# jasonleebrown/machisplin

Hardware: AMD Instinct MI355X
Metric: grid Mcells/s (ensemble+TPS predict) + TPS-solve GFLOP/s (higher is better)
Workload: dtype f64; 1 GPU; cfg3: 5000 stations, 3 covariates, 10000x10000 grid, 6-model ensemble + TPS residual correction; stations=5000, covariates=3 x float32 planes resident in HBM, rf_trees=500, tps_mode=global (one fit on all stations, GCV lambda, V73:748-753), parallelism=rowband1 + bcast(coef) + 1 all-gather

## Files before the change

include/machisplin_hip.h:

```cpp
#ifndef MACHISPLIN_HIP_H
#define MACHISPLIN_HIP_H

#include <stdint.h>

#if defined(__GNUC__)
#define MHS_API __attribute__((visibility("default")))
#else
#define MHS_API
#endif

#ifdef __cplusplus
extern "C" {
#endif

enum {
    MHS_OK = 0,
    MHS_ERR_INVALID = 1,
    MHS_ERR_HIP = 2,
    MHS_ERR_NODEVICE = 3,
    MHS_ERR_NUMERIC = 4,
    MHS_ERR_ALLOC = 5
};

enum { MHS_F64 = 0, MHS_F32 = 1, MHS_I16 = 2 };
// ... 88 lines not shown
MHS_API int mhs_nnet_fit_many(int count, const double *const *X, const double *const *y, const int64_t *n, int p, int size,
                              double *const *wts, int maxit, double abstol, double reltol, double *value, int *counts,
                              int *fail);
MHS_API int mhs_nnet_load(const double *wts, int p, int size, double y_scale, double y_shift,
                          mhs_model **out);
MHS_API int mhs_earth_load(const double *coef, const int32_t *dirs, const double *cuts, int nterms,
                           int p, mhs_model **out);
MHS_API int mhs_svr_load(const double *alpha, const double *sv, int64_t nsv, int p, double b,
                         double sigma, const double *x_center, const double *x_scale,
                         double y_center, double y_scale, mhs_model **out);
MHS_API int mhs_gbm_load(double init_f, int64_t n_trees, const int64_t *tree_offsets,
                         const int32_t *split_var, const double *split_val, const int32_t *left,
                         const int32_t *right, const int32_t *missing, int p, mhs_model **out);
MHS_API int mhs_gbm_grow_many(int count, const double *const *X, const double *const *y, const int64_t *n, int p,
                              const int32_t *const *bags, const int64_t *bag_size, int n_new, int interaction_depth,
                              int n_minobsinnode, double shrinkage, int first_call, double *const *F, double *init_f,
                              int64_t *const *tree_offsets, int32_t *const *split_var, double *const *split_val,
                              int32_t *const *left, int32_t *const *right, int32_t *const *missing);
MHS_API int mhs_gbm_grow_many_reduction(int count, const double *const *X, const double *const *y, const int64_t *n, int p,
                                        const int32_t *const *bags, const int64_t *bag_size, int n_new, int interaction_depth,
                                        int n_minobsinnode, double shrinkage, int first_call, double *const *F, double *init_f,
                                        int64_t *const *tree_offsets, int32_t *const *split_var, double *const *split_val,
                                        int32_t *const *left, int32_t *const *right, int32_t *const *missing,
                                        double *const *error_reduction);
MHS_API int mhs_rf_load(int64_t n_trees, const int64_t *tree_offsets, const int32_t *left,
                        const int32_t *right, const int32_t *status, const int32_t *best_var,
                        const double *split, const double *node_pred, int p, mhs_model **out);
MHS_API int mhs_rf_fit_many(int count, const double *const *X, const double *const *y, const int64_t *n, int p,
                            int n_trees, int mtry, int nodesize, const int32_t *const *inbag,
                            const uint64_t *const *seeds, mhs_model **models_out, double *const *oob_pred,
                            int32_t *const *oob_count, double *const *inc_node_purity);
MHS_API int mhs_rf_get(const mhs_model *m, int64_t *n_nodes, int32_t *left, int32_t *right, int32_t *status,
                       int32_t *best_var, double *split, double *node_pred, int64_t *tree_offsets);
MHS_API int mhs_rf_importance_many(int count, const mhs_model *const *models, const double *const *X,
                                   const double *const *y, const int64_t *n, int p, const int32_t *const *inbag,
                                   const uint64_t *const *perm_seeds, int n_perm, double *const *inc_mse,
                                   double *const *inc_mse_sd, double *const *tree_delta);
#define MHS_EARTH_MAX_NK 65
#define MHS_EARTH_STOP_CONSTANT 1
#define MHS_EARTH_STOP_NK 2
#define MHS_EARTH_STOP_NONE 3
#define MHS_EARTH_STOP_THRESH 4
#define MHS_EARTH_STOP_RSQ 5
#define MHS_EARTH_STOP_GRSQ 6
MHS_API int mhs_earth_fit_many(int count, const double *const *X, const double *const *y, const int64_t *n, int p,
                               int nk , double thresh, double penalty, int minspan, int endspan,
                               mhs_model **models_out);
MHS_API int mhs_earth_get(const mhs_model *m, int *n_selected, int *n_forward, int *stop_reason, double *coef,
                          int32_t *dirs, double *cuts, int32_t *forward_dirs, double *forward_cuts, double *forward_rss,
                          int32_t *selected, double *rss_per_subset, double *gcv_per_subset, int32_t *prune_terms,
                          double *stats);
MHS_API int mhs_model_free(mhs_model *m);

typedef struct mhs_stack {
    const void *data;
    int32_t n_layers;
    int32_t dtype;
    int64_t plane_stride;
    int64_t ld;
    double nodata;
} mhs_stack;

MHS_API int mhs_predict_dev(const mhs_model *m, const mhs_grid *g, const mhs_stack *covars,
                            int64_t r0, int64_t r1, int64_t c0, int64_t c1, double weight,
                            int accumulate, double *out_dev, int64_t ld, void *stream);
MHS_API int mhs_members_predict_dev(const mhs_model *const *models, const double *weights, int n_models,
// ... 226 lines not shown
```

machisplin_amd/_lib.py:

```python
from __future__ import annotations

import atexit
import ctypes as C
import os
import threading

_HERE = os.path.dirname(os.path.abspath(__file__))
LIB_PATH = os.path.join(_HERE, "libmachisplin_hip.so")

OK, ERR_INVALID, ERR_HIP, ERR_NODEVICE, ERR_NUMERIC, ERR_ALLOC = range(6)
F64, F32, I16 = 0, 1, 2
GCV_FIELDS, GCV_CONVERGED = 0, 1


class MhsError(RuntimeError):
    def __init__(self, code: int, msg: str):
        super().__init__(f"[mhs status {code}] {msg}")
        self.code = code


class Grid(C.Structure):
    _fields_ = [("xmin", C.c_double), ("ymax", C.c_double), ("xres", C.c_double),
                ("yres", C.c_double), ("nrow", C.c_int64), ("ncol", C.c_int64)]

# ... 85 lines not shown
    "mhs_tps_predict_points": (C.c_int, [_vp, _vp, _i64, _vp]),
    "mhs_tps_sigma2": (C.c_int, [_vp, _dp]),
    "mhs_tps_se_max_n": (C.c_int, [_i64, C.POINTER(_i64)]),
    "mhs_tps_se_build_mode": (C.c_int, [C.c_int]),
    "mhs_tps_se_info": (C.c_int, [_vp, C.POINTER(C.c_int), C.POINTER(C.c_double), C.POINTER(_i64)]),
    "mhs_tps_predict_se_points": (C.c_int, [_vp, _vp, _i64, C.c_double, _vp]),
    "mhs_tps_predict_se_grid": (C.c_int, [_vp, C.POINTER(Grid), _i64, _i64, _i64, _i64, C.c_double, _vp]),
    "mhs_tps_predict_se_grid_dev": (C.c_int, [_vp, C.POINTER(Grid), _i64, _i64, _i64, _i64, C.c_double, _vp, _i64, _vp]),
    "mhs_tps_eval_mode": (C.c_int, [C.c_int]),
    "mhs_tps_eval_plan": (C.c_int, [_vp, C.POINTER(C.c_int), C.POINTER(C.c_int), C.POINTER(_i64), C.POINTER(_i64)]),
    "mhs_lm_load": (C.c_int, [_vp, C.c_int, C.POINTER(_vp)]),
    "mhs_lm_fit": (C.c_int, [_vp, _vp, _i64, C.c_int, _vp]),
    "mhs_svr_fit": (C.c_int, [_vp, _vp, _i64, C.c_int, C.c_double, C.c_double, C.c_double, C.c_double, _i64, _vp, _vp, _vp, _vp,
                              _vp, _vp, _vp]),
    "mhs_nnet_fit": (C.c_int, [_vp, _vp, _i64, C.c_int, C.c_int, _vp, C.c_int, C.c_double, C.c_double, _vp, _vp, _vp]),
    "mhs_svr_fit_many": (C.c_int, [C.c_int, _vp, _vp, _vp, C.c_int, _vp, C.c_double, C.c_double, C.c_double, _i64, _i64, _vp, _vp, _vp,
                                   _vp, _vp, _vp, _vp, _vp]),
    "mhs_nnet_fit_many": (C.c_int, [C.c_int, _vp, _vp, _vp, C.c_int, C.c_int, _vp, C.c_int, C.c_double, C.c_double, _vp, _vp, _vp]),
    "mhs_nnet_load": (C.c_int, [_vp, C.c_int, C.c_int, C.c_double, C.c_double, C.POINTER(_vp)]),
    "mhs_earth_load": (C.c_int, [_vp, _vp, _vp, C.c_int, C.c_int, C.POINTER(_vp)]),
    "mhs_earth_fit_many": (C.c_int, [C.c_int, _vp, _vp, _vp, C.c_int, C.c_int, C.c_double, C.c_double, C.c_int, C.c_int, _vp]),
    "mhs_earth_get": (C.c_int, [_vp, _vp, _vp, _vp, _vp, _vp, _vp, _vp, _vp, _vp, _vp, _vp, _vp, _vp, _vp]),
    "mhs_svr_load": (C.c_int, [_vp, _vp, _i64, C.c_int, C.c_double, C.c_double, _vp, _vp, C.c_double,
                               C.c_double, C.POINTER(_vp)]),
    "mhs_gbm_load": (C.c_int, [C.c_double, _i64, _vp, _vp, _vp, _vp, _vp, _vp, C.c_int, C.POINTER(_vp)]),
    "mhs_gbm_grow_many": (C.c_int, [C.c_int, _vp, _vp, _vp, C.c_int, _vp, _vp, C.c_int, C.c_int, C.c_int, C.c_double, C.c_int, _vp, _vp,
                                    _vp, _vp, _vp, _vp, _vp, _vp]),
    "mhs_gbm_grow_many_reduction": (C.c_int, [C.c_int, _vp, _vp, _vp, C.c_int, _vp, _vp, C.c_int, C.c_int, C.c_int, C.c_double, C.c_int, _vp,
                                              _vp, _vp, _vp, _vp, _vp, _vp, _vp, _vp]),
    "mhs_rf_load": (C.c_int, [_i64, _vp, _vp, _vp, _vp, _vp, _vp, _vp, C.c_int, C.POINTER(_vp)]),
    "mhs_rf_fit_many": (C.c_int, [C.c_int, _vp, _vp, _vp, C.c_int, C.c_int, C.c_int, C.c_int, _vp, _vp, _vp, _vp, _vp, _vp]),
    "mhs_rf_get": (C.c_int, [_vp, _vp, _vp, _vp, _vp, _vp, _vp, _vp, _vp]),
    "mhs_rf_importance_many": (C.c_int, [C.c_int, _vp, _vp, _vp, _vp, C.c_int, _vp, _vp, C.c_int, _vp, _vp, _vp]),
    "mhs_model_free": (C.c_int, [_vp]),
    "mhs_predict_dev": (C.c_int, [_vp, C.POINTER(Grid), C.POINTER(Stack), _i64, _i64, _i64, _i64,
                                  C.c_double, C.c_int, _vp, _i64, _vp]),
    "mhs_members_predict_dev": (C.c_int, [C.POINTER(_vp), _dp, C.c_int, C.POINTER(Grid), C.POINTER(Stack), C.c_int64, C.c_int64,
                                          C.c_int64, C.c_int64, C.c_int, C.c_void_p, C.c_int64, C.c_void_p]),
    "mhs_ensemble_predict_dev": (C.c_int, [C.POINTER(_vp), _dp, C.c_int, C.c_double, C.POINTER(Grid),
                                           C.POINTER(Stack), _i64, _i64, _i64, _i64, _vp, _i64, _vp]),
    "mhs_ensemble_predict": (C.c_int, [C.POINTER(_vp), _dp, C.c_int, C.c_double, C.POINTER(Grid),
                                       C.POINTER(Stack), _i64, _i64, _i64, _i64, _vp]),
    "mhs_predict_points": (C.c_int, [_vp, _vp, _i64, _vp]),
    "mhs_gbm_staged_points": (C.c_int, [_vp, _vp, _i64, C.c_int, _vp]),
    "mhs_model_info": (C.c_int, [_vp, _vp, _vp, _vp]),
    "mhs_gbm_probe_last": (C.c_int, [_vp, _vp, _vp]),
    "mhs_residual_points": (C.c_int, [_vp, _vp, C.c_int, C.c_double, _vp, _vp, _i64, _vp]),
    "mhs_scale_add_dev": (C.c_int, [_vp, C.c_double, _vp, _vp, _i64, _vp]),
    "mhs_mess_create": (C.c_int, [_vp, _i64, C.c_int, C.POINTER(_vp)]),
    "mhs_mess_free": (C.c_int, [_vp]),
    "mhs_mess_grid_dev": (C.c_int, [_vp, C.POINTER(Grid), C.POINTER(Stack), _i64, _i64, _i64, _i64, _vp, _i64, _vp, _i64, _vp]),
    "mhs_mess_grid": (C.c_int, [_vp, C.POINTER(Grid), C.POINTER(Stack), _i64, _i64, _i64, _i64, _vp, _vp]),
    "mhs_mess_points": (C.c_int, [_vp, _vp, _i64, _vp, _vp]),
    "mhs_terrain_max_radius": (C.c_int, []),
    "mhs_terrain_dev": (C.c_int, [C.POINTER(Grid), C.POINTER(Stack), C.c_int, C.POINTER(TerrainUnits), _i64, _i64, _i64, _i64, C.c_uint,
                                  _vp, C.c_int, _i64, _i64, _vp]),
    "mhs_relief_dev": (C.c_int, [C.POINTER(Grid), C.POINTER(Stack), C.c_int, C.POINTER(TerrainUnits), C.c_int, _i64, _i64, _i64, _i64,
                                 C.c_uint, _vp, C.c_int, _i64, _i64, _vp]),
    "mhs_geomorphon_dev": (C.c_int, [C.POINTER(Grid), C.POINTER(Stack), C.c_int, C.POINTER(TerrainUnits), C.c_int, C.c_double, _i64, _i64,
                                     _i64, _i64, _vp, _i64, _vp]),
    "mhs_terrain": (C.c_int, [C.POINTER(Grid), C.POINTER(Stack), C.c_int, C.POINTER(TerrainUnits), _i64, _i64, _i64, _i64, C.c_uint, _vp,
                              C.c_int]),
    "mhs_relief": (C.c_int, [C.POINTER(Grid), C.POINTER(Stack), C.c_int, C.POINTER(TerrainUnits), C.c_int, _i64, _i64, _i64, _i64, C.c_uint,
                             _vp, C.c_int]),
    "mhs_geomorphon": (C.c_int, [C.POINTER(Grid), C.POINTER(Stack), C.c_int, C.POINTER(TerrainUnits), C.c_int, C.c_double, _i64, _i64, _i64,
                                 _i64, _vp]),
# ... 132 lines not shown
```

machisplin_amd/csrc/forest.hip:

```cpp
#include <type_traits>
#include <algorithm>
#include <cmath>
#include <cstdio>
#include <cstdlib>
#include <cstring>
#include <vector>
#include "ensemble_int.h"
#include "devmath.h"

namespace mhs {

constexpr int RF_COARSE_BYTES = LUT_COARSE * (int)sizeof(float);
constexpr unsigned RF_LEAF_WORD = 0xffffff00u;
typedef unsigned uint2v __attribute__((ext_vector_type(2)));
typedef unsigned uint4v __attribute__((ext_vector_type(4)));
__device__ __forceinline__ uint2v lds_u2(unsigned a) { return *(__attribute__((address_space(3))) const uint2v *)(uintptr_t)a; }
__device__ __forceinline__ unsigned lds_u32(unsigned a) { return *(__attribute__((address_space(3))) const unsigned *)(uintptr_t)a; }
__device__ __forceinline__ double lds_f64(unsigned a) { return *(__attribute__((address_space(3))) const double *)(uintptr_t)a; }

__host__ __device__ constexpr int rf_walks(int code) { return code >= 3 ? code + 2 : (1 << code); }


template <int R>
__device__ __forceinline__ void rf_lane_cells(const PredGeom &g, int64_t i0, int strips, int (&row)[R], int (&col)[R], bool (&live)[R]) {
    const int64_t total = (int64_t)g.nr * g.nc;
    const int64_t part = (total + R - 1) / R;
#pragma unroll
    for (int c = 0; c < R; ++c) {
        if (strips) {
            const int64_t sr = i0 / g.nc;
            col[c] = (int)(i0 - sr * g.nc);
            const int64_t r = sr * R + c;
            live[c] = r < g.nr;
            row[c] = (int)(live[c] ? r : g.nr - 1);
        } else {
            int64_t i = i0 + c * part;
            live[c] = i0 < part && i < total;
            if (i >= total) i = total - 1;
            row[c] = (int)(i / g.nc); col[c] = (int)(i - (int64_t)row[c] * g.nc);
        }
    }
}
static int64_t rf_lane_count(const PredGeom &g, int R, int strips) {
    const int64_t total = (int64_t)g.nr * g.nc;
    return strips ? (((int64_t)g.nr + R - 1) / R) * g.nc : (total + R - 1) / R;
}
static int rf_strips(const PredGeom &g, int R) { return g.nr >= 4 * R; }

constexpr int RF_ENTRY_BATCHES = 16;
constexpr int RF_PREFIX_MAX_P = 12;
template <int R>
__device__ __forceinline__ void rf_prefix_entries(unsigned (&entry)[RF_ENTRY_BATCHES], const uint2 *__restrict__ gnodes,
                                                  const int *__restrict__ tree_off, int n_trees, int p, const char *smem,
                                                  unsigned lane_base, const bool (&na)[R]) {
    const int lane = threadIdx.x & 63;
    int mn[RF_PREFIX_MAX_P], mx[RF_PREFIX_MAX_P];
#pragma unroll
    for (int v = 0; v < 12; ++v) {
        mn[v] = 0x7fffffff; mx[v] = -1;
        if (v < p) {
            int a = 0x7fffffff, b = -1;
#pragma unroll
            for (int c = 0; c < R; ++c)
                if (!na[c]) {
                    const int rk = (int)(*(const unsigned *)(smem + lane_base + (unsigned)(v * R + c) * 4u) >> 8);
                    a = min(a, rk); b = max(b, rk);
                }
#pragma unroll
            for (int q = 32; q > 0; q >>= 1) { a = min(a, __shfl_xor(a, q)); b = max(b, __shfl_xor(b, q)); }
            mn[v] = __builtin_amdgcn_readfirstlane(a); mx[v] = __builtin_amdgcn_readfirstlane(b);
        }
    }
#pragma unroll
    for (int b = 0; b < RF_ENTRY_BATCHES; ++b) {
        if (b * 64 < n_trees) {
            const int t = b * 64 + lane;
            bool walking = t < n_trees;
            const int o = tree_off[min(t, n_trees - 1)];
            unsigned nd = 0u, plen = 0u, term = 0u;
            while (__builtin_amdgcn_ballot_w64(walking)) {
                if (walking) {
                    const uint2 rec = gnodes[o + (int)nd];
                    if (rec.x == RF_LEAF_WORD) { term = 1u; walking = false; }
// ... 132 lines not shown
        for (int c = 0; c < R; ++c) {
            acc[c] = acc[c] + pending[c];
            pending[c] = glval[o + (int)((node[c] - boff) >> 3)];
        }
        __syncthreads();
        o = o1; o1 = o2; o2 = o3; o3 = o4;
        levels = levels1; levels1 = levels2;
        shallow = shallow1; shallow1 = shallow2;
    }
#pragma unroll
    for (int c = 0; c < R; ++c) {
        acc[c] = acc[c] + pending[c];
        if (live[c])
            emit(out, (int64_t)row[c] * g.ld_out + col[c], na[c] ? NAN : acc[c] / (double)n_trees, weight, accumulate);
    }
}

__device__ __forceinline__ void lds_wait_ge(unsigned addr, unsigned target) {
    for (;;) {
        unsigned v;
        asm volatile("ds_read_b32 %0, %1\n\ts_waitcnt lgkmcnt(0)" : "=v"(v) : "v"(addr) : "memory");
        if ((unsigned)__builtin_amdgcn_readfirstlane((int)v) >= target) break;
        __builtin_amdgcn_s_sleep(2);
    }
}
__device__ __forceinline__ void lds_signal(unsigned addr) {
    if ((threadIdx.x & 63) == 0) asm volatile("ds_add_u32 %0, %1" :: "v"(addr), "v"(1u) : "memory");
    else asm volatile("" ::: "memory");
}

__device__ __forceinline__ void glds16(const void *gsrc, unsigned lds_dst) {
    asm volatile("s_mov_b32 m0, %1\n\ts_nop 0\n\tglobal_load_lds_dwordx4 %0, off" :: "v"(gsrc), "s"(lds_dst) : "memory");
}
enum { RF_LD_PREFIX = 1 };

template <int LOG2R, bool K64, int STRIDE>
__global__ __launch_bounds__(1024) void rf_walk_ld_kernel(const uint2 *__restrict__ gnodes,
                                                          const double *__restrict__ glval,
                                                          const int *__restrict__ tree_off,
                                                          const int *__restrict__ depth,
                                                          const void *__restrict__ sorted,
                                                          const int *__restrict__ sorted_off, int n_trees,
                                                          int p, StackDev s, PredGeom g,
                                                          double weight, int accumulate,
                                                          double *__restrict__ out, const int *__restrict__ dmin, int strips, int flags,
                                                          const int *__restrict__ axis_rank, int axis_ncol) {
    constexpr int R = rf_walks(LOG2R), NL = 1, WALKERS = 16 - NL;
    constexpr unsigned TREE_BYTES = 3u * STRIDE;
    static_assert(TREE_BYTES >= (unsigned)RF_COARSE_BYTES && 2 * STRIDE <= 65535, "buffer bases inside the 16-bit immediate offsets");
    constexpr unsigned CNT = TREE_BYTES;
    extern __shared__ __attribute__((aligned(16))) char smem[];
    float *coarse = (float *)smem;
    const unsigned stride = (unsigned)(p * R) | 1u;
    const unsigned lane_base = TREE_BYTES + 32u + threadIdx.x * stride * 4u;
    if ((unsigned)(uintptr_t)(__attribute__((address_space(3))) char *)smem != 0u) __builtin_trap();
    const bool loader = threadIdx.x >= 64 * WALKERS;
    const int64_t i0 = (int64_t)blockIdx.x * (64 * WALKERS) + (loader ? threadIdx.x - 64 * WALKERS : threadIdx.x);
    int row[R], col[R];
    bool na[R], live[R];
    if (strips == 2) {
        const int wave = (int)(threadIdx.x >> 6), lane_ = (int)(threadIdx.x & 63u);
        const int64_t tile = (int64_t)blockIdx.x * WALKERS + (loader ? wave - WALKERS : wave);
        const int tiles_x = (g.nc + 15) / 16;
        const int64_t ty = tile / tiles_x;
        const int tx = (int)(tile - ty * tiles_x);
#pragma unroll
        for (int c = 0; c < R; ++c) {
            const int64_t r = ty * (4 * R) + (lane_ >> 4) * R + c;
            const int cc = tx * 16 + (lane_ & 15);
            live[c] = r < g.nr && cc < g.nc;
            row[c] = (int)min(r, (int64_t)g.nr - 1); col[c] = min(cc, g.nc - 1);
        }
    } else
    rf_lane_cells<R>(g, i0, strips, row, col, live);
#pragma unroll
    for (int c = 0; c < R; ++c) na[c] = false;
    for (int j = 0; j < p; ++j) {
        float r[R];
        if (axis_rank && j >= s.C && !s.all_from_planes) {
#pragma unroll
            for (int c = 0; c < R; ++c)
                r[c] = (float)(j == s.C ? axis_rank[g.c0 + col[c]] : axis_rank[(int64_t)axis_ncol + g.r0 + row[c]]);
        } else if constexpr (K64) lut_ranks_t<R, 1024, double>(j, (const double *)sorted, sorted_off, (double *)coarse, s, g, row, col, na, r);
        else lut_ranks_t<R, 1024, float>(j, (const float *)sorted, sorted_off, coarse, s, g, row, col, na, r);
#pragma unroll
        for (int c = 0; c < R; ++c) *(unsigned *)(smem + lane_base + (unsigned)(j * R + c) * 4u) = (unsigned)r[c] << 8;
    }
    unsigned entry[RF_ENTRY_BATCHES];
#pragma unroll
    for (int b = 0; b < RF_ENTRY_BATCHES; ++b) entry[b] = 0u;
    if (!loader && (flags & RF_LD_PREFIX) && p <= RF_PREFIX_MAX_P && n_trees <= 64 * RF_ENTRY_BATCHES)
        rf_prefix_entries<R>(entry, gnodes, tree_off, n_trees, p, smem, lane_base, na);
    __syncthreads();
    if (threadIdx.x < 8) *(unsigned *)(smem + CNT + threadIdx.x * 4u) = 0u;
    __syncthreads();
    if (loader) {
        constexpr int PF = (STRIDE + 1023) / 1024;
        static_assert(PF <= 25, "one named register quad per piece below");
        const unsigned lane16 = (threadIdx.x & 63u) * 16u;
        uint4 r0, r1, r2, r3, r4, r5, r6, r7, r8, r9, r10, r11, r12, r13, r14, r15, r16, r17, r18, r19, r20, r21, r22, r23, r24;
        const char *src = nullptr;
#define MHS_RF_ALL(F) F(0) F(1) F(2) F(3) F(4) F(5) F(6) F(7) F(8) F(9) F(10) F(11) F(12) F(13) F(14) F(15) F(16) F(17) F(18) F(19) F(20) \
                      F(21) F(22) F(23) F(24)
#define MHS_RF_LOAD(Q) if constexpr (Q < PF) r##Q = *(const uint4 *)(src + (size_t)Q * 1024u);
#define MHS_RF_STORE(Q) if constexpr (Q < PF) *(uint4 *)(smem + slot * (unsigned)STRIDE + (unsigned)Q * 1024u + lane16) = r##Q;
#define MHS_RF_REQUEST(U) { \
            src = (const char *)(gnodes + tree_off[(U)]) + lane16; \
            MHS_RF_ALL(MHS_RF_LOAD) }
        {
            MHS_RF_REQUEST(0)
            for (int u = 0; u < n_trees; u += 2) {
                unsigned slot = (unsigned)u % 3u;
                if (u >= 3) lds_wait_ge(CNT + 16u + 4u * slot, (unsigned)WALKERS * (unsigned)(u / 3));
                MHS_RF_ALL(MHS_RF_STORE)
                lds_signal(CNT + 4u * slot);
                if (u + 2 < n_trees) MHS_RF_REQUEST(u + 2)
                if (u + 1 < n_trees) {
                    slot = (unsigned)(u + 1) % 3u;
                    if (u + 1 >= 3) lds_wait_ge(CNT + 16u + 4u * slot, (unsigned)WALKERS * (unsigned)((u + 1) / 3));
                    {
                        const char *dsrc = (const char *)(gnodes + tree_off[u + 1]) + lane16;
#pragma unroll
                        for (int q = 0; q < PF; ++q)
                            glds16(dsrc + (size_t)q * 1024u, (unsigned)__builtin_amdgcn_readfirstlane((int)(slot * (unsigned)STRIDE + (unsigned)q * 1024u)));
                        asm volatile("s_waitcnt vmcnt(0)" ::: "memory");
                    }
                    lds_signal(CNT + 4u * slot);
                }
            }
            return;
        }
#undef MHS_RF_REQUEST
#undef MHS_RF_STORE
#undef MHS_RF_LOAD
#undef MHS_RF_ALL
        return;
    }
    constexpr int PD = 6;
    double acc[R], pend[PD][R];
#pragma unroll
    for (int c = 0; c < R; ++c) {
        acc[c] = 0.0;
#pragma unroll
        for (int k = 0; k < PD; ++k) pend[k][c] = 0.0;
    }
    unsigned staged[3] = {0u, 0u, 0u};
    int ocur = 0;
    unsigned wcur = 0u;
    double tpcur = 0.0;
    const int lane = threadIdx.x & 63;
    auto step = [&](auto slot_tag, auto pidx_tag, const int t, const unsigned k3) {
        constexpr int SLOT = decltype(slot_tag)::value, PIDX = decltype(pidx_tag)::value;
        if ((t & 63) == 0) {
            unsigned ecur = 0u;
#pragma unroll
            for (int b = 0; b < RF_ENTRY_BATCHES; ++b) if ((t >> 6) == b) ecur = entry[b];
            const int tl = min(t + lane, n_trees - 1);
            ocur = tree_off[tl];
            const int dcur = depth[tl], mcur = dmin ? dmin[tl] : dcur;
            const int plen = (int)((ecur >> 16) & 0x7FFFu);
            const int levels = (ecur >> 31) ? 0 : dcur - plen, shallow = max(mcur - plen, 0);
            const int c0 = min(shallow, levels - 1), cnt = levels - 1 - c0;
            wcur = ((ecur & 0xFFFFu) << 3) | (levels > 0 ? ((unsigned)c0 << 19) | ((unsigned)cnt << 25) | 0x80000000u : 0u);
            tpcur = levels > 0 ? 0.0 : glval[ocur + (int)(ecur & 0xFFFFu)];
            asm volatile("" : "+v"(ocur), "+v"(wcur), "+v"(tpcur));
        }
        const unsigned wk = (unsigned)__builtin_amdgcn_readlane((int)wcur, t & 63);
        const int o = __builtin_amdgcn_readlane(ocur, t & 63);
        if (staged[SLOT] <= k3)
            for (;;) {
                uint4v cv;
                asm volatile("ds_read_b128 %0, %1\n\ts_waitcnt lgkmcnt(0)" : "=v"(cv) : "v"(CNT) : "memory");
                staged[0] = (unsigned)__builtin_amdgcn_readfirstlane((int)cv.x);
                staged[1] = (unsigned)__builtin_amdgcn_readfirstlane((int)cv.y);
                staged[2] = (unsigned)__builtin_amdgcn_readfirstlane((int)cv.z);
                if (staged[SLOT] > k3) break;
                __builtin_amdgcn_s_sleep(1);
            }
        unsigned node[R];
#pragma unroll
        for (int c = 0; c < R; ++c) node[c] = wk & 0x7FFF8u;
        int c0 = (int)((wk >> 19) & 63u), cnt = (int)((wk >> 25) & 63u);
        if constexpr (R == 4) {
            if (wk >> 31)
                asm volatile(
#include "rf_walk_loop4xo.inc"
                    : [n0] "+v"(node[0]), [n1] "+v"(node[1]), [n2] "+v"(node[2]), [n3] "+v"(node[3]), [cnt] "+s"(cnt), [c0] "+s"(c0)
                    : [lb] "v"(lane_base), [off] "n"(SLOT * STRIDE)
                    : "memory", "vcc", "scc", "v100", "v101", "v102", "v103", "v104", "v105", "v106", "v107", "v110", "v111", "v112", "v113",
                      "v115", "v116", "v117", "v118", "v120");
        } else {
            static_assert(R == 4 || R == 5, "hand loops exist for four and five walks");
            if (wk >> 31)
                asm volatile(
#include "rf_walk_loop5xo.inc"
                    : [n0] "+v"(node[0]), [n1] "+v"(node[1]), [n2] "+v"(node[2]), [n3] "+v"(node[3]), [n4] "+v"(node[R - 1]), [cnt] "+s"(cnt),
                      [c0] "+s"(c0)
// ... 942 lines not shown
    unsigned long long z[16] = {};
    if (hipMemcpyFromSymbol(out16, HIP_SYMBOL(g_cbs_stats), sizeof(z)) != hipSuccess) return 1;
    return hipMemcpyToSymbol(HIP_SYMBOL(g_cbs_stats), z, sizeof(z)) != hipSuccess;
}
#endif


enum { RF_PICK_AUTO = 0, RF_PICK_LD, RF_PICK_DB, RF_PICK_COMPACT, RF_PICK_SUB, RF_PICK_CBS };
static int rf_pick() {
    const char *e = getenv("MHS_RF_KERNEL");
    if (!e) return RF_PICK_AUTO;
    return !strcmp(e, "ld") ? RF_PICK_LD : !strcmp(e, "db") ? RF_PICK_DB : !strcmp(e, "compact") ? RF_PICK_COMPACT : !strcmp(e, "sub") ? RF_PICK_SUB
         : !strcmp(e, "cbs") ? RF_PICK_CBS : RF_PICK_AUTO;
}
static bool rf_plain() { return getenv("MHS_RF_PLAIN") != nullptr; }

static size_t rf_walk_db_lds(const mhs_model *m, int log2r) {
    const size_t tree_bytes = std::max((size_t)m->rf_max_nodes * 16, (size_t)RF_COARSE_BYTES);
    return tree_bytes + (size_t)1024 * (((size_t)m->p * rf_walks(log2r)) | 1) * 4;
}
static int rf_walk_db_log2r(const mhs_model *m) {
    if (m->rf_max_nodes > 4095) return -1;
    for (int l2 = 3; l2 >= 1; --l2)
        if ((m->p * rf_walks(l2) * 4) <= 255 && rf_walk_db_lds(m, l2) <= LDS_LIMIT) return l2;
    return -1;
}

static bool rf_walk_ld_config(const mhs_model *m, int *log2r, int *stride) {
    if (m->rf_max_depth > 63) return false;
    for (int st : {16384, 24576, 25600}) {
        if ((size_t)m->rf_max_nodes * 8 > (size_t)st) continue;
        for (int l2 = st != 25600 ? 3 : 2; l2 >= 2; --l2)
            if ((m->p * rf_walks(l2) * 4) <= 255 &&
                (size_t)3 * st + 32 + (size_t)1024 * (((size_t)m->p * rf_walks(l2)) | 1) * 4 <= LDS_MAX) {
                *log2r = l2; *stride = st;
                return true;
            }
    }
    return false;
}

template <typename KT>
static int build_rf_nodes_t(mhs_model *m, const mhs_grid &grid, int C, int log2r, int form) {
    const bool big = form == RF_BIG;
    const size_t nn = m->rf_thr.size();
    std::vector<KT> tkey(nn, (KT)0);
    std::vector<std::vector<KT>> sorted((size_t)m->p);
    for (size_t k = 0; k < nn; ++k) {
        const unsigned v = m->rf_var[k];
        if (v == 0xFFFFu) continue;
        const KT tk = split_tkey<KT, true>((int)v, C, m->rf_thr[k], grid);
        tkey[k] = tk;
        sorted[(size_t)v].push_back(tk);
    }
    std::vector<int> off;
    std::vector<KT> flat;
    sort_unique(sorted, off, flat);
    for (int v = 0; v < m->p; ++v)
        if (sorted[(size_t)v].size() >= ((size_t)1 << 24)) { set_error("randomForest: too many distinct split values"); return MHS_ERR_INVALID; }
    if (int rc = publish_axis_ranks(m, sorted, C, grid)) return rc;
    std::vector<unsigned long long> rec((nn ? nn : 1) + 3200, 0ull);
    const unsigned R = (unsigned)rf_walks(log2r);
    if (form == RF_COMPACT) {
        rec.clear();
        std::vector<int> coff(1, 0), newid, csub, before, end;
        std::vector<double> clval;
        for (int t = 0; t < m->n_trees; ++t) {
// ... 38 lines not shown
    } else
    for (size_t k = 0; k < nn; ++k) {
        const unsigned v = m->rf_var[k];
        const unsigned left = m->rf_left[k], right = m->rf_right[k];
        const unsigned unit = big ? 1u : 8u;
        unsigned node0 = 0, children;
        if (v == 0xFFFFu) {
            children = (left * unit) | ((left * unit) << 16);
            if (!big) node0 = RF_LEAF_WORD;
        } else {
            const std::vector<KT> &sv = sorted[(size_t)v];
            const unsigned j = (unsigned)(std::lower_bound(sv.begin(), sv.end(), tkey[k]) - sv.begin());
            node0 = (j << 8) | (v * R * 4u);
            children = (left * unit) | ((right * unit) << 16);
        }
        rec[k] = ((unsigned long long)children << 32) | node0;
    }
    if (int rc = publish(m, flat, (KT **)&m->lut_sorted)) return rc;
    if (int rc = publish(m, off, &m->lut_sorted_off)) return rc;
    return publish(m, rec, &m->rf_nodes);
}

static int build_rf_nodes(mhs_model *m, const mhs_grid &grid, int C, int log2r, int form, int key64, TreeTables *tt) {
    std::lock_guard<std::mutex> lk(m->mu);
    if (!(m->rf_nodes && m->rf_log2r == log2r && m->rf_form == form && same_meta(m, grid, C, key64))) {
        if (int rc = key64 ? build_rf_nodes_t<double>(m, grid, C, log2r, form) : build_rf_nodes_t<float>(m, grid, C, log2r, form)) return rc;
        m->meta_grid = grid; m->meta_C = C; m->meta_key64 = key64;
        m->rf_log2r = log2r; m->rf_form = form;
    }
    *tt = TreeTables{m->lut_sorted, m->lut_sorted_off, nullptr, m->rf_nodes, form == RF_COMPACT ? m->rf_coff : nullptr, nullptr, nullptr, nullptr,
                     m->axis_rank, m->axis_ncol, form == RF_COMPACT ? m->rf_csub : nullptr, form == RF_COMPACT ? m->rf_clval : nullptr};
    return MHS_OK;
}

static int launch_rf_walk(const mhs_model *m, const StackDev &s, const PredGeom &g, const mhs_grid &grid,
                          double w, int acc, double *out, hipStream_t st, int64_t total, bool *launched) {
    const int key64 = s.dtype == MHS_F64, pick = rf_pick();
    *launched = false;
    (void)total;
    int sb_l2 = 0, sb_stride = 0;
    if (pick == RF_PICK_SUB && rf_walk_ld_config(m, &sb_l2, &sb_stride) && m->n_trees <= 64 * RF_ENTRY_BATCHES) {
        TreeTables tt;
        if (int rc = build_rf_nodes(const_cast<mhs_model *>(m), grid, s.C, sb_l2, RF_SMALL, key64, &tt)) return rc;
        const int R = rf_walks(sb_l2);
        const int tiles = rf_strips(g, R);
        unsigned blocks;
        if (tiles) {
            const int64_t tiles_x = (g.nc + 15) / 16, tiles_y = (g.nr + 4 * R - 1) / (4 * R);
            blocks = (unsigned)(((tiles_x + 4) / 5) * ((tiles_y + 2) / 3));
        } else blocks = (unsigned)((rf_lane_count(g, R, 0) + 64 * 15 - 1) / (64 * 15));
        const int *dmin = rf_plain() ? nullptr : m->rf_dmin;
        const size_t tbytes = (size_t)3 * sb_stride + 64 + (size_t)1024 * (((size_t)m->p * R) | 1) * 4;
#define MHS_SB(L2, ST) (key64 ? rf_walk_sub_kernel<L2, true, ST> : rf_walk_sub_kernel<L2, false, ST>)
        auto tk = sb_stride == 16384 ? (sb_l2 == 3 ? MHS_SB(3, 16384) : MHS_SB(2, 16384))
                : sb_stride == 24576 ? (sb_l2 == 3 ? MHS_SB(3, 24576) : MHS_SB(2, 24576))
                                     : MHS_SB(2, 25600);
#undef MHS_SB
        if (tbytes <= LDS_MAX) {
            MHS_HIP(hipFuncSetAttribute((const void *)tk, hipFuncAttributeMaxDynamicSharedMemorySize, (int)tbytes));
            hipLaunchKernelGGL(tk, dim3(blocks), dim3(1024), tbytes, st, (const uint2 *)tt.rf_nodes, m->rf_lval, m->tree_off,
                               m->rf_depth, tt.sorted, tt.sorted_off, m->n_trees, m->p, s, g, w, acc, out, dmin, tiles,
                               (int)(tiles && dmin), tt.axis_rank, tt.axis_ncol);
            *launched = true;
            return MHS_OK;
        }
    }
    int ld_l2 = 0, ld_stride = 0;
    if (pick != RF_PICK_DB && rf_walk_ld_config(m, &ld_l2, &ld_stride)) {
        TreeTables tt;
        if (int rc = build_rf_nodes(const_cast<mhs_model *>(m), grid, s.C, ld_l2, RF_SMALL, key64, &tt)) return rc;
        const int R = rf_walks(ld_l2);
        const int strips = rf_strips(g, R);
        const int64_t per_block = 64 * 15;
        unsigned blocks = (unsigned)((rf_lane_count(g, R, strips) + per_block - 1) / per_block);
        if (strips) blocks = (unsigned)((((int64_t)(g.nc + 15) / 16) * ((g.nr + 4 * R - 1) / (4 * R)) + 15 - 1) / 15);
        const int *dmin = rf_plain() ? nullptr : m->rf_dmin;
        const size_t tbytes = (size_t)3 * ld_stride + 32 + (size_t)1024 * (((size_t)m->p * R) | 1) * 4;
#define MHS_LD(L2, ST) (key64 ? rf_walk_ld_kernel<L2, true, ST> : rf_walk_ld_kernel<L2, false, ST>)
        auto tk = ld_stride == 16384 ? (ld_l2 == 3 ? MHS_LD(3, 16384) : MHS_LD(2, 16384))
                : ld_stride == 24576 ? (ld_l2 == 3 ? MHS_LD(3, 24576) : MHS_LD(2, 24576))
                                     : MHS_LD(2, 25600);
#undef MHS_LD
        MHS_HIP(hipFuncSetAttribute((const void *)tk, hipFuncAttributeMaxDynamicSharedMemorySize, (int)tbytes));
        hipLaunchKernelGGL(tk, dim3(blocks), dim3(1024), tbytes, st, (const uint2 *)tt.rf_nodes, m->rf_lval, m->tree_off,
                           m->rf_depth, tt.sorted, tt.sorted_off, m->n_trees, m->p, s, g, w, acc, out, dmin, strips ? 2 : 0,
                           (int)(strips && dmin), tt.axis_rank, tt.axis_ncol);
        *launched = true;
        return MHS_OK;
    }
    const int log2r = rf_walk_db_log2r(m);
    if (log2r < 0) return MHS_OK;
    TreeTables tt;
    if (int rc = build_rf_nodes(const_cast<mhs_model *>(m), grid, s.C, log2r, RF_SMALL, key64, &tt)) return rc;
    const int R = rf_walks(log2r);
    const size_t dbytes = rf_walk_db_lds(m, log2r);
    const int strips = rf_strips(g, R);
    const unsigned blocks = (unsigned)((rf_lane_count(g, R, strips) + 1023) / 1024);
    const int *dmin = rf_plain() ? nullptr : m->rf_dmin;
    auto dk = log2r == 3 ? (key64 ? rf_walk_db_kernel<3, true> : rf_walk_db_kernel<3, false>)
            : log2r == 2 ? (key64 ? rf_walk_db_kernel<2, true> : rf_walk_db_kernel<2, false>)
                         : (key64 ? rf_walk_db_kernel<1, true> : rf_walk_db_kernel<1, false>);
    MHS_HIP(hipFuncSetAttribute((const void *)dk, hipFuncAttributeMaxDynamicSharedMemorySize, (int)dbytes));
    hipLaunchKernelGGL(dk, dim3(blocks), dim3(1024), dbytes, st, (const uint2 *)tt.rf_nodes, m->rf_lval, m->tree_off,
                       m->rf_depth, tt.sorted, key64, tt.sorted_off, m->n_trees, m->rf_max_nodes, m->p, s, g, w, acc, out, dmin, strips,
                       strips && dmin);
    *launched = true;
    return MHS_OK;
}

static int rf_compact_threads(const mhs_model *m) {
    if (!m->rf_compact_ok || m->p * 16 > 255) return 0;
    const size_t tree_bytes = std::max((size_t)m->rf_cmax * 8, (size_t)RF_COARSE_BYTES);
    if (tree_bytes >= LDS_MAX) return 0;
    const size_t per_lane = (((size_t)m->p * 4) | 1) * 4;
    int nt = (int)std::min<size_t>(1024, (LDS_MAX - tree_bytes) / per_lane) / 64 * 64;
    if (nt < 512 || (size_t)nt * 8 < (size_t)m->rf_cmax) return 0;
    return nt;
}

// ... 184 lines not shown
            }
            depth[(size_t)t] = dmax;
            m->rf_max_depth = std::max(m->rf_max_depth, dmax);
            shallow[(size_t)t] = std::min(dlow, dmax);
        }
        if (paired) {
            m->rf_off.push_back((int)nodes.size());
            m->rf_compact_ok = 1;
            for (int64_t t = 0; t < n_trees; ++t) {
                int splits = 0;
                for (int k = m->rf_off[(size_t)t]; k < m->rf_off[(size_t)t + 1]; ++k) splits += m->rf_var[(size_t)k] != 0xFFFFu;
                m->rf_cmax = std::max(m->rf_cmax, splits + 1);
                if (8 * splits + (m->rf_off[(size_t)t + 1] - m->rf_off[(size_t)t]) > 65535) m->rf_compact_ok = 0;
            }
            m->rf_fast = true;
            m->rf_max_nodes = max_nodes;
            int rc = to_device(lval.data(), lval.size(), &m->rf_lval);
            if (!rc) rc = to_device(depth.data(), depth.size(), &m->rf_depth);
            if (!rc) rc = to_device(shallow.data(), shallow.size(), &m->rf_dmin);
            if (rc) { mhs_model_free(m); return rc; }
        }
    }
    m->slot = current_slot(); m->device = ctx().device;
    m->reload = [n_trees, to = std::vector<int64_t>(tree_offsets, tree_offsets + n_trees + 1), l = std::vector<int32_t>(left, left + nn),
                 r = std::vector<int32_t>(right, right + nn), st = std::vector<int32_t>(status, status + nn),
                 bv = std::vector<int32_t>(best_var, best_var + nn), sp = std::vector<double>(split, split + nn),
                 np_ = std::vector<double>(node_pred, node_pred + nn), p](mhs_model **o) {
        return mhs_rf_load(n_trees, to.data(), l.data(), r.data(), st.data(), bv.data(), sp.data(), np_.data(), p, o);
    };
    *out = m;
    return MHS_OK;
}

}
```

Before: 414.2 Mcells/s.

## Skip staging RF trees whose prefix already resolves every lane in the block

The LDS-staged random-forest walk now has walkers vote, using wave ballots and LDS atomics, on which trees still need walking after the prefix-entry step. The loader wave only copies those trees' node tables into shared memory and skips the DMA for the rest. This cuts global-to-LDS traffic and wait time for trees already resolved to a leaf. In exchange it adds per-block ballot, atomic and barrier work, a larger LDS header, an env override to stage everything, and an optional skip counter API.

```diff
diff --git a/include/machisplin_hip.h b/include/machisplin_hip.h
--- a/include/machisplin_hip.h
+++ b/include/machisplin_hip.h
@@ -144,6 +144,7 @@
                             int32_t *const *oob_count, double *const *inc_node_purity);
 MHS_API int mhs_rf_get(const mhs_model *m, int64_t *n_nodes, int32_t *left, int32_t *right, int32_t *status,
                        int32_t *best_var, double *split, double *node_pred, int64_t *tree_offsets);
+MHS_API int mhs_rf_stage_skip_stats(int enable, int64_t *skipped);
 MHS_API int mhs_rf_importance_many(int count, const mhs_model *const *models, const double *const *X,
                                    const double *const *y, const int64_t *n, int p, const int32_t *const *inbag,
                                    const uint64_t *const *perm_seeds, int n_perm, double *const *inc_mse,
diff --git a/machisplin_amd/_lib.py b/machisplin_amd/_lib.py
--- a/machisplin_amd/_lib.py
+++ b/machisplin_amd/_lib.py
@@ -141,6 +141,7 @@
     "mhs_rf_fit_many": (C.c_int, [C.c_int, _vp, _vp, _vp, C.c_int, C.c_int, C.c_int, C.c_int, _vp, _vp, _vp, _vp, _vp, _vp]),
     "mhs_rf_get": (C.c_int, [_vp, _vp, _vp, _vp, _vp, _vp, _vp, _vp, _vp]),
     "mhs_rf_importance_many": (C.c_int, [C.c_int, _vp, _vp, _vp, _vp, C.c_int, _vp, _vp, C.c_int, _vp, _vp, _vp]),
+    "mhs_rf_stage_skip_stats": (C.c_int, [C.c_int, C.POINTER(C.c_int64)]),
     "mhs_model_free": (C.c_int, [_vp]),
     "mhs_predict_dev": (C.c_int, [_vp, C.POINTER(Grid), C.POINTER(Stack), _i64, _i64, _i64, _i64,
                                   C.c_double, C.c_int, _vp, _i64, _vp]),
diff --git a/machisplin_amd/csrc/forest.hip b/machisplin_amd/csrc/forest.hip
--- a/machisplin_amd/csrc/forest.hip
+++ b/machisplin_amd/csrc/forest.hip
@@ -49,6 +49,10 @@
 
 constexpr int RF_ENTRY_BATCHES = 16;
 constexpr int RF_PREFIX_MAX_P = 12;
+__device__ __forceinline__ int rf_levels_left(unsigned entry, int depth) {
+    return (entry >> 31) ? 0 : depth - (int)((entry >> 16) & 0x7FFFu);
+}
+__device__ __forceinline__ bool rf_wave_walks(unsigned entry, int depth) { return rf_levels_left(entry, depth) > 0; }
 template <int R>
 __device__ __forceinline__ void rf_prefix_entries(unsigned (&entry)[RF_ENTRY_BATCHES], const uint2 *__restrict__ gnodes,
                                                   const int *__restrict__ tree_off, int n_trees, int p, const char *smem,
@@ -247,7 +251,8 @@
 __device__ __forceinline__ void glds16(const void *gsrc, unsigned lds_dst) {
     asm volatile("s_mov_b32 m0, %1\n\ts_nop 0\n\tglobal_load_lds_dwordx4 %0, off" :: "v"(gsrc), "s"(lds_dst) : "memory");
 }
-enum { RF_LD_PREFIX = 1 };
+enum { RF_LD_PREFIX = 1, RF_LD_STAGE_ALL = 2 };
+constexpr unsigned RF_LD_HEAD = 32u + 8u * RF_ENTRY_BATCHES;
 
 template <int LOG2R, bool K64, int STRIDE>
 __global__ __launch_bounds__(1024) void rf_walk_ld_kernel(const uint2 *__restrict__ gnodes,
@@ -259,15 +264,16 @@
                                                           int p, StackDev s, PredGeom g,
                                                           double weight, int accumulate,
                                                           double *__restrict__ out, const int *__restrict__ dmin, int strips, int flags,
-                                                          const int *__restrict__ axis_rank, int axis_ncol) {
+                                                          const int *__restrict__ axis_rank, int axis_ncol, int *__restrict__ stats) {
     constexpr int R = rf_walks(LOG2R), NL = 1, WALKERS = 16 - NL;
     constexpr unsigned TREE_BYTES = 3u * STRIDE;
     static_assert(TREE_BYTES >= (unsigned)RF_COARSE_BYTES && 2 * STRIDE <= 65535, "buffer bases inside the 16-bit immediate offsets");
     constexpr unsigned CNT = TREE_BYTES;
+    constexpr unsigned NEED = CNT + 32u;
     extern __shared__ __attribute__((aligned(16))) char smem[];
     float *coarse = (float *)smem;
     const unsigned stride = (unsigned)(p * R) | 1u;
-    const unsigned lane_base = TREE_BYTES + 32u + threadIdx.x * stride * 4u;
+    const unsigned lane_base = TREE_BYTES + RF_LD_HEAD + threadIdx.x * stride * 4u;
     if ((unsigned)(uintptr_t)(__attribute__((address_space(3))) char *)smem != 0u) __builtin_trap();
     const bool loader = threadIdx.x >= 64 * WALKERS;
     const int64_t i0 = (int64_t)blockIdx.x * (64 * WALKERS) + (loader ? threadIdx.x - 64 * WALKERS : threadIdx.x);
@@ -290,6 +296,8 @@
     rf_lane_cells<R>(g, i0, strips, row, col, live);
 #pragma unroll
     for (int c = 0; c < R; ++c) na[c] = false;
+    if (threadIdx.x < 2 * RF_ENTRY_BATCHES) *(unsigned *)(smem + NEED + threadIdx.x * 4u) = 0u;
+    if (s.C == 0) __syncthreads();
     for (int j = 0; j < p; ++j) {
         float r[R];
         if (axis_rank && j >= s.C && !s.all_from_planes) {
@@ -304,8 +312,30 @@
     unsigned entry[RF_ENTRY_BATCHES];
 #pragma unroll
     for (int b = 0; b < RF_ENTRY_BATCHES; ++b) entry[b] = 0u;
-    if (!loader && (flags & RF_LD_PREFIX) && p <= RF_PREFIX_MAX_P && n_trees <= 64 * RF_ENTRY_BATCHES)
-        rf_prefix_entries<R>(entry, gnodes, tree_off, n_trees, p, smem, lane_base, na);
+    const bool prefix = (flags & RF_LD_PREFIX) && p <= RF_PREFIX_MAX_P && n_trees <= 64 * RF_ENTRY_BATCHES;
+    if (!loader) {
+        const bool vote = prefix && !(flags & RF_LD_STAGE_ALL);
+        const int lane_ = (int)(threadIdx.x & 63u);
+        int dep[RF_ENTRY_BATCHES];
+#pragma unroll
+        for (int b = 0; b < RF_ENTRY_BATCHES; ++b) dep[b] = 0;
+        if (vote) {
+#pragma unroll
+            for (int b = 0; b < RF_ENTRY_BATCHES; ++b) dep[b] = depth[min(b * 64 + lane_, n_trees - 1)];
+        }
+        if (prefix) rf_prefix_entries<R>(entry, gnodes, tree_off, n_trees, p, smem, lane_base, na);
+        unsigned mine = 0xffffffffu;
+        if (vote) {
+            mine = 0u;
+#pragma unroll
+            for (int b = 0; b < RF_ENTRY_BATCHES; ++b) {
+                const bool walks = b * 64 + lane_ < n_trees && rf_wave_walks(entry[b], dep[b]);
+                const unsigned long long bal = __builtin_amdgcn_ballot_w64(walks);
+                if ((lane_ >> 1) == b) mine = (lane_ & 1) ? (unsigned)(bal >> 32) : (unsigned)bal;
+            }
+        }
+        if ((threadIdx.x & 63u) < 2u * RF_ENTRY_BATCHES) atomicOr((unsigned *)(smem + NEED + (threadIdx.x & 63u) * 4u), mine);
+    }
     __syncthreads();
     if (threadIdx.x < 8) *(unsigned *)(smem + CNT + threadIdx.x * 4u) = 0u;
     __syncthreads();
@@ -319,30 +349,49 @@
                       F(21) F(22) F(23) F(24)
 #define MHS_RF_LOAD(Q) if constexpr (Q < PF) r##Q = *(const uint4 *)(src + (size_t)Q * 1024u);
 #define MHS_RF_STORE(Q) if constexpr (Q < PF) *(uint4 *)(smem + slot * (unsigned)STRIDE + (unsigned)Q * 1024u + lane16) = r##Q;
-#define MHS_RF_REQUEST(U) { \
-            src = (const char *)(gnodes + tree_off[(U)]) + lane16; \
+#define MHS_RF_REQUEST(O) { \
+            src = (const char *)(gnodes + (O)) + lane16; \
             MHS_RF_ALL(MHS_RF_LOAD) }
         {
-            MHS_RF_REQUEST(0)
+            const unsigned needv = lds_u32(NEED + (threadIdx.x & 31u) * 4u);
+            auto needed = [&](int u) -> unsigned {
+                unsigned w, in;
+                asm volatile("v_readlane_b32 %0, %2, %3\n\ts_sub_i32 %1, %5, %6\n\ts_lshr_b32 %0, %0, %4\n\ts_lshr_b32 %1, %1, 31\n\ts_and_b32 %0, %0, %1"
+                             : "=&s"(w), "=&s"(in) : "v"(needv), "s"((u >> 5) & (2 * RF_ENTRY_BATCHES - 1)), "s"(u & 31), "s"(u), "s"(n_trees) : "scc");
+                return w;
+            };
+            unsigned copied = 0u;
+            unsigned parked = needed(0);
+            unsigned dma = needed(1), request = needed(2);
+            int o_dma = tree_off[min(1, n_trees)], o_request = tree_off[min(2, n_trees)];
+            if (parked) MHS_RF_REQUEST(tree_off[0])
             for (int u = 0; u < n_trees; u += 2) {
                 unsigned slot = (unsigned)u % 3u;
                 if (u >= 3) lds_wait_ge(CNT + 16u + 4u * slot, (unsigned)WALKERS * (unsigned)(u / 3));
-                MHS_RF_ALL(MHS_RF_STORE)
+                copied += parked;
+                if (parked) { MHS_RF_ALL(MHS_RF_STORE) }
                 lds_signal(CNT + 4u * slot);
-                if (u + 2 < n_trees) MHS_RF_REQUEST(u + 2)
+                parked = request;
+                if (parked) MHS_RF_REQUEST(o_request)
                 if (u + 1 < n_trees) {
                     slot = (unsigned)(u + 1) % 3u;
                     if (u + 1 >= 3) lds_wait_ge(CNT + 16u + 4u * slot, (unsigned)WALKERS * (unsigned)((u + 1) / 3));
-                    {
-                        const char *dsrc = (const char *)(gnodes + tree_off[u + 1]) + lane16;
+                    const unsigned now = dma;
+                    copied += now;
+                    if (now) {
+                        const char *dsrc = (const char *)(gnodes + o_dma) + lane16;
 #pragma unroll
                         for (int q = 0; q < PF; ++q)
                             glds16(dsrc + (size_t)q * 1024u, (unsigned)__builtin_amdgcn_readfirstlane((int)(slot * (unsigned)STRIDE + (unsigned)q * 1024u)));
-                        asm volatile("s_waitcnt vmcnt(0)" ::: "memory");
                     }
+                    dma = needed(u + 3); request = needed(u + 4);
+                    o_dma = tree_off[min(u + 3, n_trees)]; o_request = tree_off[min(u + 4, n_trees)];
+                    if (now) asm volatile("s_waitcnt vmcnt(0)" ::: "memory");
                     lds_signal(CNT + 4u * slot);
                 }
             }
+            const int skipped = n_trees - (int)copied;
+            if (stats && (threadIdx.x & 63u) == 0 && skipped) atomicAdd(stats, skipped);
             return;
         }
 #undef MHS_RF_REQUEST
@@ -374,10 +423,11 @@
             ocur = tree_off[tl];
             const int dcur = depth[tl], mcur = dmin ? dmin[tl] : dcur;
             const int plen = (int)((ecur >> 16) & 0x7FFFu);
-            const int levels = (ecur >> 31) ? 0 : dcur - plen, shallow = max(mcur - plen, 0);
+            const int levels = rf_levels_left(ecur, dcur), shallow = max(mcur - plen, 0);
+            const bool walks = rf_wave_walks(ecur, dcur);
             const int c0 = min(shallow, levels - 1), cnt = levels - 1 - c0;
-            wcur = ((ecur & 0xFFFFu) << 3) | (levels > 0 ? ((unsigned)c0 << 19) | ((unsigned)cnt << 25) | 0x80000000u : 0u);
-            tpcur = levels > 0 ? 0.0 : glval[ocur + (int)(ecur & 0xFFFFu)];
+            wcur = ((ecur & 0xFFFFu) << 3) | (walks ? ((unsigned)c0 << 19) | ((unsigned)cnt << 25) | 0x80000000u : 0u);
+            tpcur = walks ? 0.0 : glval[ocur + (int)(ecur & 0xFFFFu)];
             asm volatile("" : "+v"(ocur), "+v"(wcur), "+v"(tpcur));
         }
         const unsigned wk = (unsigned)__builtin_amdgcn_readlane((int)wcur, t & 63);
@@ -1386,7 +1436,7 @@
         if ((size_t)m->rf_max_nodes * 8 > (size_t)st) continue;
         for (int l2 = st != 25600 ? 3 : 2; l2 >= 2; --l2)
             if ((m->p * rf_walks(l2) * 4) <= 255 &&
-                (size_t)3 * st + 32 + (size_t)1024 * (((size_t)m->p * rf_walks(l2)) | 1) * 4 <= LDS_MAX) {
+                (size_t)3 * st + RF_LD_HEAD + (size_t)1024 * (((size_t)m->p * rf_walks(l2)) | 1) * 4 <= LDS_MAX) {
                 *log2r = l2; *stride = st;
                 return true;
             }
@@ -1491,6 +1541,8 @@
                      m->axis_rank, m->axis_ncol, form == RF_COMPACT ? m->rf_csub : nullptr, form == RF_COMPACT ? m->rf_clval : nullptr};
     return MHS_OK;
 }
+
+static std::atomic<int *> g_rf_skip_stats{nullptr};
 
 static int launch_rf_walk(const mhs_model *m, const StackDev &s, const PredGeom &g, const mhs_grid &grid,
                           double w, int acc, double *out, hipStream_t st, int64_t total, bool *launched) {
@@ -1534,7 +1586,9 @@
         unsigned blocks = (unsigned)((rf_lane_count(g, R, strips) + per_block - 1) / per_block);
         if (strips) blocks = (unsigned)((((int64_t)(g.nc + 15) / 16) * ((g.nr + 4 * R - 1) / (4 * R)) + 15 - 1) / 15);
         const int *dmin = rf_plain() ? nullptr : m->rf_dmin;
-        const size_t tbytes = (size_t)3 * ld_stride + 32 + (size_t)1024 * (((size_t)m->p * R) | 1) * 4;
+        const size_t tbytes = (size_t)3 * ld_stride + RF_LD_HEAD + (size_t)1024 * (((size_t)m->p * R) | 1) * 4;
+        const char *sa = getenv("MHS_RF_STAGE_ALL");
+        const int ld_flags = (strips && dmin ? RF_LD_PREFIX : 0) | (sa && atoi(sa) ? RF_LD_STAGE_ALL : 0);
 #define MHS_LD(L2, ST) (key64 ? rf_walk_ld_kernel<L2, true, ST> : rf_walk_ld_kernel<L2, false, ST>)
         auto tk = ld_stride == 16384 ? (ld_l2 == 3 ? MHS_LD(3, 16384) : MHS_LD(2, 16384))
                 : ld_stride == 24576 ? (ld_l2 == 3 ? MHS_LD(3, 24576) : MHS_LD(2, 24576))
@@ -1543,7 +1597,7 @@
         MHS_HIP(hipFuncSetAttribute((const void *)tk, hipFuncAttributeMaxDynamicSharedMemorySize, (int)tbytes));
         hipLaunchKernelGGL(tk, dim3(blocks), dim3(1024), tbytes, st, (const uint2 *)tt.rf_nodes, m->rf_lval, m->tree_off,
                            m->rf_depth, tt.sorted, tt.sorted_off, m->n_trees, m->p, s, g, w, acc, out, dmin, strips ? 2 : 0,
-                           (int)(strips && dmin), tt.axis_rank, tt.axis_ncol);
+                           ld_flags, tt.axis_rank, tt.axis_ncol, g_rf_skip_stats.load());
         *launched = true;
         return MHS_OK;
     }
@@ -1794,4 +1848,30 @@
     return MHS_OK;
 }
 
-}
+int mhs_rf_stage_skip_stats(int enable, int64_t *skipped) {
+    if (int rc = require_ready()) return rc;
+    int *cnt = g_rf_skip_stats.load();
+    if (skipped) {
+        *skipped = 0;
+        if (cnt) {
+            int v = 0;
+            MHS_HIP(hipDeviceSynchronize());
+            MHS_HIP(hipMemcpy(&v, cnt, sizeof(int), hipMemcpyDeviceToHost));
+            MHS_HIP(hipMemset(cnt, 0, sizeof(int)));
+            *skipped = v;
+        }
+    }
+    if (enable && !cnt) {
+        MHS_HIP(hipMalloc(&cnt, sizeof(int)));
+        MHS_HIP(hipMemset(cnt, 0, sizeof(int)));
+        MHS_HIP(hipDeviceSynchronize());
+        g_rf_skip_stats.store(cnt);
+    } else if (!enable && cnt) {
+        g_rf_skip_stats.store(nullptr);
+        MHS_HIP(hipDeviceSynchronize());
+        MHS_HIP(hipFree(cnt));
+    }
+    return MHS_OK;
+}
+
+}
```

Result: no change. 414.6 Mcells/s (median of 3 runs) (+0.1%).
